# cucibala/FaceRecognizeOnnx

Measured on AMD Instinct MI355X. Metric: faces/sec end-to-end (detect+align+embed), batch=128 640x640, higher is better.
Workload: dtype f32; 1 GPU; C-headline: 128 frames 640x640 per GPU, SCRFD det_500m + decode + NMS, first 1 face(s)/frame aligned to 112x112, IResNet-50 (w600k_r50) embed, L2-norm; frames_per_gpu=128, faces_per_frame=1, weights=synthetic seeded (det seed 100, rec seed 200), input_residency=HBM-resident before the timed region, gallery_rows=0, topk=0, parallelism=frame-sharded x1, no data-path collective

## Files before the change

facerecognizeonnx_amd/csrc/conv_wino2.hip:

```cpp
#include <hip/hip_runtime.h>

#include <algorithm>
#include <cstdlib>
#include <cstring>
#include <stdexcept>
#include <vector>

#include "gemm_tile.h"
#include "kernels.h"
#include "plan.h"

namespace fh {

namespace {

__device__ __forceinline__ float act1(float v, bool relu, float sl) {
    const float a = v >= 0.f ? v : v * sl;
    return relu ? fmaxf(v, 0.f) : a;
}

constexpr int kYA[4] = {0, 1, 2, 1}, kYB[4] = {2, 2, 1, 3};
constexpr int kSA[4] = {1, 1, 1, 1}, kSB[4] = {-1, 1, -1, -1};
constexpr int kAT[2][4] = {{1, 1, 1, 0}, {0, 1, -1, -1}};

template <int V> struct IC { static constexpr int value = V; };

template <int CB, int NW, bool MERGED>
__global__ __launch_bounds__(64 * NW, NW == 1 ? 2 : 3) void wino2_kernel(const ConvArgs p, const int tiles_n, const int tgx, const int tgy, const int n_tg) {
    extern __shared__ v4f w2sm[];
    char* const halo = reinterpret_cast<char*>(w2sm);
    const int lane = threadIdx.x & 63;
    const int wv = NW == 1 ? 0 : __builtin_amdgcn_readfirstlane((int)threadIdx.x >> 6);
    constexpr int CBT = CB * NW;
#ifdef FACEHIP_W2_PROF
    const long long prof_c0 = __builtin_readcyclecounter(), prof_r0 = __builtin_amdgcn_s_memrealtime();
#endif
    int blk;
    {
        const int n = gridDim.x, q = n >> 3, r = n & 7, x = blockIdx.x & 7;
        blk = x * q + min(x, r) + (int)(blockIdx.x >> 3);
    }
    const int tile_n = blk % tiles_n, tg = blk / tiles_n;
    const int H = p.H, W = p.W;
    const int per_img = tgx * tgy;
    const int gn = tg / per_img, rem = tg - gn * per_img;
    const int gy = rem / tgx, gx = rem - gy * tgx;
    (void)n_tg;
    const int tn = lane & 15, kq = lane >> 4, tr = tn >> 2, tc = tn & 3;
    auto key = [](int pr, int pc) { return 2 * ((pc + 4 * (pr & 1)) & 7); };

    {
        const int col = lane & 15, pl = lane >> 4;
        const int y0 = 8 * gy - 1 + (pl >> 1), x0 = 8 * gx - 1 + (pl & 1);
        const float* const img = p.in + ((size_t)gn * H * W + (size_t)y0 * W + x0) * 64;
#pragma unroll
        for (int i = 0; i < 25; ++i) {
            const int pr = i / 5, pc = i - 5 * pr;
            const int y = y0 + 2 * pr, x = x0 + 2 * pc;
            const bool ok = (unsigned)y < (unsigned)H && (unsigned)x < (unsigned)W;
            if (NW > 1 && (i % NW) != wv) continue;
            lds_dma16(ok ? img + ((long)2 * pr * W + 2 * pc) * 64 + ((col ^ key(pr, pc)) << 2) : p.zeros, halo + i * 1024);
        }
    }
    typedef const __attribute__((address_space(3))) v4f* lds_v4f;
    const unsigned halo_base = (unsigned)(size_t)(__attribute__((address_space(3))) char*)halo;
    unsigned rb[16];
#pragma unroll
    for (int dy = 0; dy < 4; ++dy)
#pragma unroll
        for (int dx = 0; dx < 4; ++dx) {
            const int pl = (dy & 1) * 2 + (dx & 1), pr = tr + (dy >> 1), pc = tc + (dx >> 1);
            rb[dy * 4 + dx] = halo_base + (unsigned)((4 * (pr * 5 + pc) + pl) * 256 + ((key(pr, pc) ^ kq) << 4));
        }
    const char* wstep = reinterpret_cast<const char*>(p.wt + ((size_t)tile_n * 64 * CBT + (size_t)wv * CB) * 256);
    const unsigned wlane = lane * 16;
    constexpr int WD = 2;
    v4f wr[WD][CB] = {};
#ifdef FACEHIP_W2_PROF
    const bool abl_w = p.sk_test_drop & 4, abl_d = p.sk_test_drop & 8, abl_y = p.sk_test_drop & 16, abl_st = p.sk_test_drop & 2;
#else
    constexpr bool abl_w = false, abl_d = false, abl_y = false, abl_st = false;
#endif
    auto fetch_w = [&](bool advance, int buf) __attribute__((always_inline)) {
        if (abl_w) return;
        unsigned adv = advance ? CBT * 1024 : 0;
        asm volatile("" : "+s"(adv));
        wstep += adv;
#pragma unroll
        for (int cb = 0; cb < CB; ++cb) wr[buf][cb] = *reinterpret_cast<const v4f*>(wstep + wlane + cb * 1024);
    };
    v4f Y[2][2][CB], Mp[CB];
#pragma unroll
    for (int cb = 0; cb < CB; ++cb) {
        Mp[cb] = v4f{0.f, 0.f, 0.f, 0.f};
#pragma unroll
        for (int a = 0; a < 4; ++a) Y[a >> 1][a & 1][cb] = v4f{0.f, 0.f, 0.f, 0.f};
    }
    auto y_update = [&](auto fc, const v4f (&M)[CB]) __attribute__((always_inline)) {
        constexpr int f = decltype(fc)::value, i = f >> 2, j = f & 3;
        if (abl_y && f != 5) return;
        constexpr int c00 = kAT[0][i] * kAT[0][j], c01 = kAT[0][i] * kAT[1][j], c10 = kAT[1][i] * kAT[0][j], c11 = kAT[1][i] * kAT[1][j];
#pragma unroll
        for (int cb = 0; cb < CB; ++cb) {
            if constexpr (c00 > 0) Y[0][0][cb] += M[cb]; else if constexpr (c00 < 0) Y[0][0][cb] -= M[cb];
            if constexpr (c01 > 0) Y[0][1][cb] += M[cb]; else if constexpr (c01 < 0) Y[0][1][cb] -= M[cb];
            if constexpr (c10 > 0) Y[1][0][cb] += M[cb]; else if constexpr (c10 < 0) Y[1][0][cb] -= M[cb];
            if constexpr (c11 > 0) Y[1][1][cb] += M[cb]; else if constexpr (c11 < 0) Y[1][1][cb] -= M[cb];
            if constexpr (c00 != 0) asm volatile("" : "+v"(Y[0][0][cb]));
            if constexpr (c01 != 0) asm volatile("" : "+v"(Y[0][1][cb]));
            if constexpr (c10 != 0) asm volatile("" : "+v"(Y[1][0][cb]));
            if constexpr (c11 != 0) asm volatile("" : "+v"(Y[1][1][cb]));
        }
    };
    v4f d[2][4] = {};
    auto fetch_d = [&](auto fc, auto jc, auto bc) __attribute__((always_inline)) {
        constexpr int f = decltype(fc)::value, j = decltype(jc)::value, buf = decltype(bc)::value;
        constexpr int fi = f >> 2, fj = f & 3;
        constexpr int ya = kYA[fi], yb = kYB[fi], xa = kYA[fj], xb = kYB[fj];
        if (abl_d) return;
        unsigned gxr = j << 6;
        asm volatile("" : "+s"(gxr));
        d[buf][0] = *reinterpret_cast<lds_v4f>((size_t)(rb[ya * 4 + xa] ^ gxr));
        d[buf][1] = *reinterpret_cast<lds_v4f>((size_t)(rb[ya * 4 + xb] ^ gxr));
        d[buf][2] = *reinterpret_cast<lds_v4f>((size_t)(rb[yb * 4 + xa] ^ gxr));
        d[buf][3] = *reinterpret_cast<lds_v4f>((size_t)(rb[yb * 4 + xb] ^ gxr));
    };
    auto stage = [&](auto fc) __attribute__((always_inline)) {
        constexpr int f = decltype(fc)::value;
        constexpr int fi = f >> 2, fj = f & 3;
        constexpr int sab = kSA[fi] * kSB[fj], sba = kSB[fi] * kSA[fj], sbb = kSB[fi] * kSB[fj];
        v4f M[CB];
#pragma unroll
        for (int cb = 0; cb < CB; ++cb) M[cb] = v4f{0.f, 0.f, 0.f, 0.f};
        auto step = [&](auto jc) __attribute__((always_inline)) {
            constexpr int j = decltype(jc)::value, k = f * 4 + j;
            fetch_w(k + WD - 1 < 64, (k + WD - 1) % WD);
            if constexpr (j < 3) fetch_d(IC<f>{}, IC<j + 1>{}, IC<(k + 1) & 1>{});
            else if constexpr (f < 15) fetch_d(IC<f + 1>{}, IC<0>{}, IC<(k + 1) & 1>{});
            __builtin_amdgcn_sched_barrier(0);
            const v4f* dd = d[k & 1];
            v4f v = dd[0];
            v = sab > 0 ? v + dd[1] : v - dd[1];
            v = sba > 0 ? v + dd[2] : v - dd[2];
            v = sbb > 0 ? v + dd[3] : v - dd[3];
            asm volatile("" : "+v"(v));
            __builtin_amdgcn_sched_barrier(0);
#pragma unroll
            for (int e = 0; e < 4; ++e)
#pragma unroll
                for (int cb = 0; cb < CB; ++cb) M[cb] = __builtin_amdgcn_mfma_f32_16x16x4f32(wr[k % WD][cb][e], v[e], M[cb], 0, 0, 0);
            __builtin_amdgcn_sched_barrier(0);
        };
        step(IC<0>{}); step(IC<1>{});
        y_update(IC<(f + 15) & 15>{}, Mp);
        step(IC<2>{}); step(IC<3>{});
#pragma unroll
        for (int cb = 0; cb < CB; ++cb) Mp[cb] = M[cb];
        __builtin_amdgcn_sched_barrier(0);
    };
    fetch_w(false, 0);
#pragma unroll
    for (int q = 1; q < WD - 1; ++q) fetch_w(true, q);
    asm volatile("s_waitcnt vmcnt(0)" ::: "memory");
    if constexpr (NW > 1) __syncthreads();
    fetch_d(IC<0>{}, IC<0>{}, IC<0>{});
    stage(IC<0>{}); stage(IC<1>{}); stage(IC<2>{}); stage(IC<3>{}); stage(IC<4>{}); stage(IC<5>{}); stage(IC<6>{}); stage(IC<7>{});
    stage(IC<8>{}); stage(IC<9>{}); stage(IC<10>{}); stage(IC<11>{}); stage(IC<12>{}); stage(IC<13>{}); stage(IC<14>{}); stage(IC<15>{});
    y_update(IC<15>{}, Mp);

    asm volatile("" ::: "memory");
    __builtin_amdgcn_sched_barrier(0);
    if (abl_st && lane != 0) return;
    const int oy0 = 2 * (4 * gy + tr), ox0 = 2 * (4 * gx + tc);
    const int n0 = (tile_n * NW + wv) * 16 * CB, Cout = p.Cout;
    const float* __restrict__ res = p.res;
    float* __restrict__ out1 = p.out1;
    float* __restrict__ out2 = p.out2;
    const bool relu = p.act == (int)Act::RELU, prelu = p.act == (int)Act::PRELU;
    float bm[CB][4];
    if constexpr (MERGED) {
#pragma unroll
        for (int cb = 0; cb < CB; ++cb)
#pragma unroll
            for (int e = 0; e < 4; ++e) { const int co = n0 + 16 * cb + 4 * kq + e; bm[cb][e] = co < Cout ? p.bias[co] : 0.f; }
    }
#pragma unroll
    for (int a = 0; a < 2; ++a)
#pragma unroll
        for (int b = 0; b < 2; ++b) {
            const int oy = oy0 + a, ox = ox0 + b;
            if (!MERGED || oy >= p.Ho || ox >= p.Wo) continue;
            const size_t pix = ((size_t)gn * p.Ho + oy) * p.Wo + ox;
            if constexpr (MERGED) {
#pragma unroll
                for (int cb = 0; cb < CB; ++cb)
#pragma unroll
                    for (int e = 0; e < 4; e += 2) {
                        const int co = n0 + 16 * cb + 4 * kq + e;
                        if (co >= Cout) continue;
                        const int g = co >= p.oc0[2] && p.n_outs > 2 ? 2 : co >= p.oc0[1] ? 1 : 0;
                        const int cg = p.oc0[g + 1] - p.oc0[g], ga = p.oact[g];
                        auto fin = [&](float v) { return ga == (int)Act::RELU ? fmaxf(v, 0.f) : ga == (int)Act::SIGMOID ? 1.0f / (1.0f + expf(-v)) : v; };
                        float* const dst = p.outs[g] + pix * cg + (co - p.oc0[g]);
                        const float v0 = fin(Y[a][b][cb][e] + bm[cb][e]);
                        if (co + 1 < p.oc0[g + 1] && !((cg | (co - p.oc0[g])) & 1)) {
                            *reinterpret_cast<float2*>(dst) = float2{v0, fin(Y[a][b][cb][e + 1] + bm[cb][e + 1])};
                        } else {
                            dst[0] = v0;
                            if (co + 1 < Cout) {
                                const int g1 = co + 1 >= p.oc0[2] && p.n_outs > 2 ? 2 : co + 1 >= p.oc0[1] ? 1 : 0;
                                const int cg1 = p.oc0[g1 + 1] - p.oc0[g1], ga1 = p.oact[g1];
                                float v1 = Y[a][b][cb][e + 1] + bm[cb][e + 1];
                                v1 = ga1 == (int)Act::RELU ? fmaxf(v1, 0.f) : ga1 == (int)Act::SIGMOID ? 1.0f / (1.0f + expf(-v1)) : v1;
                                p.outs[g1][pix * cg1 + (co + 1 - p.oc0[g1])] = v1;
                            }
                        }
                    }
                continue;
            }
        }
    if constexpr (!MERGED) {
        const int n0 = (tile_n * NW + wv) * 16 * CB + 4 * kq;
        bool live[4]; size_t row[4]; v4f b4[4][CB], r4[4][CB], sl[CB];
#pragma unroll
        for (int cb = 0; cb < CB; ++cb) sl[cb] = prelu ? *reinterpret_cast<const v4f*>(p.slope + n0 + 16 * cb) : v4f{1.f, 1.f, 1.f, 1.f};
#pragma unroll
        for (int q = 0; q < 4; ++q) {
            const int oy = oy0 + (q >> 1), ox = ox0 + (q & 1);
            live[q] = oy < p.Ho && ox < p.Wo;
            const int oyc = min(oy, p.Ho - 1), oxc = min(ox, p.Wo - 1);
            row[q] = (((size_t)gn * p.Ho + oyc) * p.Wo + oxc) * Cout + n0;
            const int cls = p.bias_cls ? 3 * (oyc == 0 ? 0 : oyc == p.Ho - 1 ? 2 : 1) + (oxc == 0 ? 0 : oxc == p.Wo - 1 ? 2 : 1) : 0;
#pragma unroll
            for (int cb = 0; cb < CB; ++cb) {
                b4[q][cb] = p.bias ? *reinterpret_cast<const v4f*>(p.bias + cls * Cout + n0 + 16 * cb) : v4f{0.f, 0.f, 0.f, 0.f};
                if (p.res_mode != (int)ResMode::NONE) r4[q][cb] = *reinterpret_cast<const v4f*>(res + row[q] + 16 * cb);
            }
        }
#pragma unroll
        for (int q = 0; q < 4; ++q) {
            if (!live[q]) continue;
#pragma unroll
            for (int cb = 0; cb < CB; ++cb) {
                v4f v;
#pragma unroll
                for (int e = 0; e < 4; ++e) v[e] = act1(Y[q >> 1][q & 1][cb][e] + b4[q][cb][e], relu, sl[cb][e]);
                if (p.res_mode != (int)ResMode::NONE) v += r4[q][cb];
                if (out1) *reinterpret_cast<v4f*>(out1 + row[q] + 16 * cb) = v;
                if (out2) {
                    const v4f s2 = *reinterpret_cast<const v4f*>(p.s2 + n0 + 16 * cb), t2 = *reinterpret_cast<const v4f*>(p.t2 + n0 + 16 * cb);
                    *reinterpret_cast<v4f*>(out2 + row[q] + 16 * cb) = v * s2 + t2;
                }
            }
        }
    }
#ifdef FACEHIP_W2_PROF
    if (lane == 0 && p.slabs && blockIdx.x < (1u << 17)) {
        const long long dc = __builtin_readcyclecounter() - prof_c0, dr = (long long)__builtin_amdgcn_s_memrealtime() - prof_r0;
        reinterpret_cast<float*>(p.slabs)[blockIdx.x] = (float)(dc * 1000 / (dr + 1));
    }
#endif
}

bool shape_ok(int Cin, int Cout) { return Cin == 64 && (Cout % 64 == 0 || Cout <= 32); }

template <int CB, int NW, bool MERGED>
void launch_cb(const ConvArgs& a, hipStream_t s) {
    const int tgy = ((a.H + 1) / 2 + 3) / 4, tgx = ((a.W + 1) / 2 + 3) / 4;
    const long n_tg = (long)a.B * tgy * tgx;
    const int tiles_n = (a.Cout + 16 * CB * NW - 1) / (16 * CB * NW);
    static const bool lds_ok = [] {
        hipFuncAttributes fa{};
        FH_HIP(hipFuncGetAttributes(&fa, reinterpret_cast<const void*>(&wino2_kernel<CB, NW, MERGED>)));
        return fa.sharedSizeBytes % 256 == 0;
    }();
    if (!lds_ok) throw std::runtime_error("wino2: static LDS moved the halo off its 256-byte alignment (see the address XOR in fetch_d)");
    KernelTimer& timer = KernelTimer::get();
    timer.begin(s);
    hipLaunchKernelGGL((wino2_kernel<CB, NW, MERGED>), dim3((unsigned)(n_tg * tiles_n)), dim3(64 * NW), 25600, s, a, tiles_n, tgx, tgy, (int)n_tg);
    timer.end(s, 12, 2.0 * 16 * 16.0 * (double)n_tg * a.Cin * (16.0 * CB * NW * tiles_n), a.t_flops);
}

}

size_t wino2_weight_floats(int Cin, int Cout) { return (size_t)16 * Cin * (Cout <= 32 ? 32 : Cout); }
void wino2_pack_weights(const float* w, int Cout, int Cin, float* dst) {
    static const double Gm[4][3] = {{1, 0, 0}, {.5, .5, .5}, {.5, -.5, .5}, {0, 0, 1}};
    if (!shape_ok(Cin, Cout)) throw std::runtime_error("wino2_pack_weights: layer shape not supported");
    const int CB = Cout <= 32 ? 2 : 4;
    memset(dst, 0, wino2_weight_floats(Cin, Cout) * sizeof(float));
    for (int co = 0; co < Cout; ++co)
        for (int ci = 0; ci < Cin; ++ci) {
            double g[3][3], t[4][3];
            for (int k = 0; k < 9; ++k) g[k / 3][k % 3] = w[((size_t)co * 9 + k) * Cin + ci];
            for (int i = 0; i < 4; ++i)
                for (int x = 0; x < 3; ++x) t[i][x] = Gm[i][0] * g[0][x] + Gm[i][1] * g[1][x] + Gm[i][2] * g[2][x];
            const int tn = co / (16 * CB), cb = (co % (16 * CB)) / 16, m = co % 16;
            const int j = ci / 16, kq = (ci % 16) / 4, e = ci % 4;
            for (int i = 0; i < 4; ++i)
                for (int jj = 0; jj < 4; ++jj) {
                    const double u = t[i][0] * Gm[jj][0] + t[i][1] * Gm[jj][1] + t[i][2] * Gm[jj][2];
                    const size_t step = ((size_t)tn * 16 + (i * 4 + jj)) * 4 + j;
                    dst[(step * CB + cb) * 256 + (kq * 16 + m) * 4 + e] = (float)u;
                }
        }
}

bool wino2_ok(const ConvArgs& a) {
    if (!(a.ks == 3 && a.stride == 1 && a.pad == 1 && a.H == a.Ho && a.W == a.Wo && a.H >= 2 && a.W >= 2 && shape_ok(a.Cin, a.Cout) &&
          a.act != (int)Act::SIGMOID && !a.sc_in && !a.dw_w && !a.u8_src && a.wt_group_rows == 0 &&
          (a.res_mode == (int)ResMode::NONE || a.res_mode == (int)ResMode::SAME)))
        return false;
    if (a.n_outs > 0)
        return a.Cout <= 32 && a.res_mode == (int)ResMode::NONE && !a.out2 && !a.bias_cls;
    return a.Cout % 64 == 0;
}

static float* g_w2_clock = nullptr;
double wino2_debug_clock_mhz() {
    if (!g_w2_clock) return 0.0;
    std::vector<float> h(1 << 17);
    if (hipMemcpy(h.data(), g_w2_clock, h.size() * sizeof(float), hipMemcpyDeviceToHost) != hipSuccess) return 0.0;
    std::vector<float> v;
    for (float x : h) if (x > 0.f) v.push_back(x);
    if (v.empty()) return 0.0;
    std::nth_element(v.begin(), v.begin() + v.size() / 2, v.end());
    return v[v.size() / 2] / 10.0;
}

long wino2_blocks(const ConvArgs& a) {
    return (long)a.B * (((a.H + 1) / 2 + 3) / 4) * (((a.W + 1) / 2 + 3) / 4) * ((a.Cout + 63) / 64) / 4;
}

void launch_wino2(const ConvArgs& a_in, hipStream_t s) {
    if (!wino2_ok(a_in)) throw std::runtime_error("launch_wino2: layer shape not supported");
    ConvArgs a = a_in;
    a.zeros = conv_zero_line();
    static const int ablate = [] { const char* e = getenv("FACEHIP_W2_ABLATE"); return e ? atoi(e) : -1; }();
    a.sk_test_drop = ablate < 0 ? 0 : ablate;
    if (ablate >= 0 && !g_w2_clock) { void* q = nullptr; if (hipMalloc(&q, sizeof(float) << 17) == hipSuccess) g_w2_clock = (float*)q; }
    if (g_w2_clock) (void)hipMemsetAsync(g_w2_clock, 0, sizeof(float) << 17, s);
    a.slabs = g_w2_clock;
    static const int nw = [] { const char* e = getenv("FACEHIP_WINO2_NW"); return e ? atoi(e) : 2; }();
    if (a.Cout <= 32) launch_cb<2, 1, true>(a, s);
    else if (nw == 2) launch_cb<2, 2, false>(a, s);
    else launch_cb<4, 1, false>(a, s);
}

}
```

Before: 12290 faces/s.

## Restructure Winograd F(2,3) input transform to share row sums across columns

The Winograd kernel's loop order changes from frequency-major to row/channel-group/column order. Each group now loads two full 4-wide input rows and computes the row-combined vector once. All four column frequencies are then derived from it, instead of doing four LDS loads and three adds per step. Four accumulators are kept live across a row, and the weight packing order is permuted to match. This cuts LDS reads and VALU transform work per MFMA step, at the cost of more registers, which risks lowering occupancy or causing spills.

```diff
diff --git a/facerecognizeonnx_amd/csrc/conv_wino2.hip b/facerecognizeonnx_amd/csrc/conv_wino2.hip
--- a/facerecognizeonnx_amd/csrc/conv_wino2.hip
+++ b/facerecognizeonnx_amd/csrc/conv_wino2.hip
@@ -20,7 +20,7 @@
 }
 
 constexpr int kYA[4] = {0, 1, 2, 1}, kYB[4] = {2, 2, 1, 3};
-constexpr int kSA[4] = {1, 1, 1, 1}, kSB[4] = {-1, 1, -1, -1};
+constexpr int kSB[4] = {-1, 1, -1, -1};
 constexpr int kAT[2][4] = {{1, 1, 1, 0}, {0, 1, -1, -1}};
 
 template <int V> struct IC { static constexpr int value = V; };
@@ -89,12 +89,11 @@
 #pragma unroll
         for (int cb = 0; cb < CB; ++cb) wr[buf][cb] = *reinterpret_cast<const v4f*>(wstep + wlane + cb * 1024);
     };
-    v4f Y[2][2][CB], Mp[CB];
+    v4f Y[2][2][CB], M[4][CB];
 #pragma unroll
     for (int cb = 0; cb < CB; ++cb) {
-        Mp[cb] = v4f{0.f, 0.f, 0.f, 0.f};
-#pragma unroll
-        for (int a = 0; a < 4; ++a) Y[a >> 1][a & 1][cb] = v4f{0.f, 0.f, 0.f, 0.f};
+#pragma unroll
+        for (int a = 0; a < 4; ++a) Y[a >> 1][a & 1][cb] = M[a][cb] = v4f{0.f, 0.f, 0.f, 0.f};
     }
     auto y_update = [&](auto fc, const v4f (&M)[CB]) __attribute__((always_inline)) {
         constexpr int f = decltype(fc)::value, i = f >> 2, j = f & 3;
@@ -113,60 +112,57 @@
         }
     };
     v4f d[2][4] = {};
-    auto fetch_d = [&](auto fc, auto jc, auto bc) __attribute__((always_inline)) {
-        constexpr int f = decltype(fc)::value, j = decltype(jc)::value, buf = decltype(bc)::value;
-        constexpr int fi = f >> 2, fj = f & 3;
-        constexpr int ya = kYA[fi], yb = kYB[fi], xa = kYA[fj], xb = kYB[fj];
+    auto fetch_d = [&](auto ic, auto gc) __attribute__((always_inline)) {
+        constexpr int i = decltype(ic)::value, g = decltype(gc)::value;
+        constexpr int ya = kYA[i], yb = kYB[i];
         if (abl_d) return;
-        unsigned gxr = j << 6;
+        unsigned gxr = g << 6;
         asm volatile("" : "+s"(gxr));
-        d[buf][0] = *reinterpret_cast<lds_v4f>((size_t)(rb[ya * 4 + xa] ^ gxr));
-        d[buf][1] = *reinterpret_cast<lds_v4f>((size_t)(rb[ya * 4 + xb] ^ gxr));
-        d[buf][2] = *reinterpret_cast<lds_v4f>((size_t)(rb[yb * 4 + xa] ^ gxr));
-        d[buf][3] = *reinterpret_cast<lds_v4f>((size_t)(rb[yb * 4 + xb] ^ gxr));
-    };
-    auto stage = [&](auto fc) __attribute__((always_inline)) {
-        constexpr int f = decltype(fc)::value;
-        constexpr int fi = f >> 2, fj = f & 3;
-        constexpr int sab = kSA[fi] * kSB[fj], sba = kSB[fi] * kSA[fj], sbb = kSB[fi] * kSB[fj];
-        v4f M[CB];
-#pragma unroll
-        for (int cb = 0; cb < CB; ++cb) M[cb] = v4f{0.f, 0.f, 0.f, 0.f};
+#pragma unroll
+        for (int x = 0; x < 4; ++x) {
+            d[0][x] = *reinterpret_cast<lds_v4f>((size_t)(rb[ya * 4 + x] ^ gxr));
+            d[1][x] = *reinterpret_cast<lds_v4f>((size_t)(rb[yb * 4 + x] ^ gxr));
+        }
+    };
+    auto group = [&](auto ic, auto gc) __attribute__((always_inline)) {
+        constexpr int i = decltype(ic)::value, g = decltype(gc)::value;
+        v4f R[4];
+#pragma unroll
+        for (int x = 0; x < 4; ++x) R[x] = kSB[i] > 0 ? d[0][x] + d[1][x] : d[0][x] - d[1][x];
+#pragma unroll
+        for (int x = 0; x < 4; ++x) asm volatile("" : "+v"(R[x]));
+        __builtin_amdgcn_sched_barrier(0);
+        if constexpr (g < 3) fetch_d(IC<i>{}, IC<g + 1>{});
+        else if constexpr (i < 3) fetch_d(IC<i + 1>{}, IC<0>{});
         auto step = [&](auto jc) __attribute__((always_inline)) {
-            constexpr int j = decltype(jc)::value, k = f * 4 + j;
+            constexpr int j = decltype(jc)::value, k = (i * 4 + g) * 4 + j;
+            if constexpr (g == 0 && i > 0) y_update(IC<(i - 1) * 4 + j>{}, M[j]);
             fetch_w(k + WD - 1 < 64, (k + WD - 1) % WD);
-            if constexpr (j < 3) fetch_d(IC<f>{}, IC<j + 1>{}, IC<(k + 1) & 1>{});
-            else if constexpr (f < 15) fetch_d(IC<f + 1>{}, IC<0>{}, IC<(k + 1) & 1>{});
             __builtin_amdgcn_sched_barrier(0);
-            const v4f* dd = d[k & 1];
-            v4f v = dd[0];
-            v = sab > 0 ? v + dd[1] : v - dd[1];
-            v = sba > 0 ? v + dd[2] : v - dd[2];
-            v = sbb > 0 ? v + dd[3] : v - dd[3];
+            v4f v = kSB[j] > 0 ? R[kYA[j]] + R[kYB[j]] : R[kYA[j]] - R[kYB[j]];
             asm volatile("" : "+v"(v));
             __builtin_amdgcn_sched_barrier(0);
 #pragma unroll
             for (int e = 0; e < 4; ++e)
 #pragma unroll
-                for (int cb = 0; cb < CB; ++cb) M[cb] = __builtin_amdgcn_mfma_f32_16x16x4f32(wr[k % WD][cb][e], v[e], M[cb], 0, 0, 0);
+                for (int cb = 0; cb < CB; ++cb)
+                    M[j][cb] = __builtin_amdgcn_mfma_f32_16x16x4f32(wr[k % WD][cb][e], v[e], g == 0 && e == 0 ? v4f{0.f, 0.f, 0.f, 0.f} : M[j][cb], 0, 0, 0);
             __builtin_amdgcn_sched_barrier(0);
         };
-        step(IC<0>{}); step(IC<1>{});
-        y_update(IC<(f + 15) & 15>{}, Mp);
-        step(IC<2>{}); step(IC<3>{});
-#pragma unroll
-        for (int cb = 0; cb < CB; ++cb) Mp[cb] = M[cb];
-        __builtin_amdgcn_sched_barrier(0);
+        step(IC<0>{}); step(IC<1>{}); step(IC<2>{}); step(IC<3>{});
+    };
+    auto row = [&](auto ic) __attribute__((always_inline)) {
+        constexpr int i = decltype(ic)::value;
+        group(IC<i>{}, IC<0>{}); group(IC<i>{}, IC<1>{}); group(IC<i>{}, IC<2>{}); group(IC<i>{}, IC<3>{});
     };
     fetch_w(false, 0);
 #pragma unroll
     for (int q = 1; q < WD - 1; ++q) fetch_w(true, q);
     asm volatile("s_waitcnt vmcnt(0)" ::: "memory");
     if constexpr (NW > 1) __syncthreads();
-    fetch_d(IC<0>{}, IC<0>{}, IC<0>{});
-    stage(IC<0>{}); stage(IC<1>{}); stage(IC<2>{}); stage(IC<3>{}); stage(IC<4>{}); stage(IC<5>{}); stage(IC<6>{}); stage(IC<7>{});
-    stage(IC<8>{}); stage(IC<9>{}); stage(IC<10>{}); stage(IC<11>{}); stage(IC<12>{}); stage(IC<13>{}); stage(IC<14>{}); stage(IC<15>{});
-    y_update(IC<15>{}, Mp);
+    fetch_d(IC<0>{}, IC<0>{});
+    row(IC<0>{}); row(IC<1>{}); row(IC<2>{}); row(IC<3>{});
+    y_update(IC<12>{}, M[0]); y_update(IC<13>{}, M[1]); y_update(IC<14>{}, M[2]); y_update(IC<15>{}, M[3]);
 
     asm volatile("" ::: "memory");
     __builtin_amdgcn_sched_barrier(0);
@@ -300,7 +296,7 @@
             for (int i = 0; i < 4; ++i)
                 for (int jj = 0; jj < 4; ++jj) {
                     const double u = t[i][0] * Gm[jj][0] + t[i][1] * Gm[jj][1] + t[i][2] * Gm[jj][2];
-                    const size_t step = ((size_t)tn * 16 + (i * 4 + jj)) * 4 + j;
+                    const size_t step = (((size_t)tn * 4 + i) * 4 + j) * 4 + jj;
                     dst[(step * CB + cb) * 256 + (kq * 16 + m) * 4 + e] = (float)u;
                 }
         }
```

After: 12400 faces/s (median of 6 runs). Within noise of the previous version (+0.9%).
